# yitian97/SDformerFlow

Hardware: AMD Instinct MI355X
Metric: event-frames/sec fwd (1x10x2x288x384) (higher is better)
Workload: dtype f16x2

## Files before the change

include/sdformerflow_hip.h:

```cpp
#ifndef SDFORMERFLOW_HIP_H
#define SDFORMERFLOW_HIP_H

#include <stdint.h>

#ifdef __cplusplus
extern "C" {
#endif

#define SDF_VERSION 107

enum { SDF_F32 = 0, SDF_U8 = 1 };
enum { SDF_LIF = 0, SDF_PSN = 1, SDF_IF = 2 };
enum {
  SDF_E_NULL = -1,
  SDF_E_SHAPE = -2,
  SDF_E_DTYPE = -3,
  SDF_E_ALIGN = -4
};

int sdf_version(void);

void sdf_switches_reload(void);

typedef struct SdfLaunchRecord {
// ... 207 lines not shown

typedef struct SdfSpikeDeconvDesc {
  const uint8_t* spikes;
  const int8_t* digits; const float* cscale;
  const float* alpha; const float* beta;
  float* out;
  int32_t imgs, T, H, W, Cin, Cout;
} SdfSpikeDeconvDesc;

int sdf_spike_deconv3x3s2_fwd(const SdfSpikeDeconvDesc* d, void* stream);

typedef struct SdfSpikeConvDesc {
  SdfSpikeGemmDesc g;
  int32_t H, W, Cin, OH, OW;
  int32_t KH, KW, sy, sx;
  int32_t dy[3], dx[3];
} SdfSpikeConvDesc;

int sdf_spike_conv2d_fwd(const SdfSpikeConvDesc* c, void* stream);
int sdf_spike_conv2d_multi_fwd(const SdfSpikeConvDesc* cs, int n, void* stream);

int sdf_split_weight_bf16(const float* W, uint16_t* planes, int64_t n, int nsplit, void* stream);

int sdf_split_weight_f16x2(const float* W, uint16_t* planes, int64_t n, float scale, void* stream);

int sdf_qk_gate_fwd(const uint8_t* q, const uint8_t* k, uint8_t* e, int Tq, int64_t rows, int C,
                    int kind, float tau, float v_th, float v_reset, int soft_reset,
                    const float* psn_w, const float* psn_b, void* stream);
int sdf_qk_gate_strided_fwd(const uint8_t* q, const uint8_t* k, uint8_t* e, int Tq, int64_t rows, int C,
                            int64_t ldq, int64_t ldk, int kind, float tau, float v_th, float v_reset,
                            int soft_reset, const float* psn_w, const float* psn_b, void* stream);

typedef struct SdfHeadConvDesc {
  const float* x;
  const float* w;
  const float* alpha;
  const float* beta;
  uint8_t* out;
  int32_t B, T, H, W, Cin, Cout;
  int32_t sn_kind;
  float tau, v_th, v_reset;
  int32_t soft_reset;
  const float* psn_w;
  const float* psn_b;
  int64_t x_sb, x_st, x_sy, x_sx;
  int64_t x_sc[4];
} SdfHeadConvDesc;

int sdf_head_conv_sn_fwd(const SdfHeadConvDesc* d, void* stream);

typedef struct SdfPointwiseConvDesc {
  const float* x;
  const float* w;
  const float* bias;
  float* out;
  int32_t imgs, H, W, Cin, N, stride, OH, OW;
} SdfPointwiseConvDesc;

int sdf_pointwise_conv_f32_fwd(const SdfPointwiseConvDesc* d, void* stream);

int sdf_deconv_col2im_fwd(const float* Y, const float* alpha, const float* beta, float* out, int imgs, int H, int W,
                          int Cout, void* stream);

int sdf_flow_out_fwd(const float* pred, float* out, int B, int D, int h, int w, int64_t ldp, int C, int H, int W,
                     float scale_y, float scale_x, void* stream);

typedef struct SdfPredHeadDesc {
  const float* z;
  int32_t B, D, h, w, Cin;
  SdfNeuronCfg sn_pred;
  const float* wgt;
  const float* bias;
  float* pred;
  float* flow;
  int32_t H, W;
  uint8_t* next_spikes;
  int32_t next_ld, next_z_off, next_pred_off, next_zero_off, next_zero_len;
  SdfNeuronCfg sn_next;
  uint8_t* keep_spikes;
} SdfPredHeadDesc;

int sdf_pred_head_fwd(const SdfPredHeadDesc* d, void* stream);

int sdf_affine_resid_fwd(const float* x, const float* alpha, const float* beta, const float* resid, float* out,
                         int64_t n, int C, int64_t inner, void* stream);

enum { SDF_ATTN_ANN = 0, SDF_ATTN_SEW = 1 };
typedef struct SdfWinAttnDesc {
  int32_t mode;
  const void* q;
  const void* k;
  const void* v;
  float* out;
  int32_t B_, nW, nH, N, hd;
  int32_t Tq, N1;
  const float* scale;
  const float* bias;
  const float* mask;
  const int32_t* row_map;
  const float* pad_qkv;
} SdfWinAttnDesc;

int sdf_win_attn_fwd(const SdfWinAttnDesc* d, void* stream);

typedef struct SdfAnnAttnBlockDesc {
  const float* x;
  float* out;
  const int32_t* row_map;
  int32_t B_, nW, nH, N, C;
  int64_t rows;
  const float* ln_w;
  const float* ln_b;
  float ln_eps;
  const uint16_t* wqkv;
  const float* qkv_bias;
  const float* scale;
  const float* table;
  const uint16_t* wproj;
  const float* proj_bias;
} SdfAnnAttnBlockDesc;

int sdf_ann_attn_block_supported(int C, int nH, int N);
int sdf_ann_attn_block_fwd(const SdfAnnAttnBlockDesc* d, void* stream);

typedef struct SdfAnnMlpBlockDesc {
  const float* x;
  float* out;
  int64_t rows;
  int32_t C, Ch;
  const float* ln_w;
  const float* ln_b;
  float ln_eps;
  const uint16_t* w1;
  const float* b1;
  const uint16_t* w2;
  const float* b2;
} SdfAnnMlpBlockDesc;

int sdf_ann_mlp_block_supported(int C, int Ch);
int sdf_ann_mlp_block_fwd(const SdfAnnMlpBlockDesc* d, void* stream);

typedef struct SdfDenseConvDesc {
  const void* x;
  const uint16_t* w;
  const float* alpha;
  const float* beta;
  const void* resid;
  void* out;
  int32_t imgs, H, W, cin_records, N;
  int32_t relu;
  int32_t out_f32;
  int32_t x_records;
  float acc_scale;
} SdfDenseConvDesc;

int sdf_dense_conv3x3_fwd(const SdfDenseConvDesc* d, void* stream);
int sdf_pack_planes(const float* x, void* planes, int imgs, int C, int H, int W, void* stream);
int sdf_unpack_planes(const void* planes, float* x, int imgs, int C, int H, int W, void* stream);
int sdf_pack_planes_up2(const float* x, void* planes, int imgs, int C, int h, int w, int64_t sn, int64_t sc, int64_t sh, int64_t sw,
                        int rec0, int rec_total, void* stream);
int sdf_pack_planes_zero_up2(const float* x, void* planes, int imgs, int C, int h, int w, int64_t sn, int64_t sc, int64_t sh, int64_t sw,
                             int rec0, int rec_total, void* stream);

typedef struct SdfDenseLinearDesc {
  const float* a;
  const uint16_t* w;
// ... 45 lines not shown
```

sdformerflow_amd/csrc/pred_head.hip:

```cpp
#include "spike_mm.h"

namespace {
using sdfmm::neuron_T;

struct PredParams {
  SdfPredHeadDesc d;
  float inv_tau_p, inv_tau_n;
  int64_t P;
  int same_next;
};

template <int T, int LPP, int NK>
__global__ __launch_bounds__(256) void pred_head_kernel(PredParams P) {
  constexpr int Cin = 12 * LPP, PPW = 64 / LPP;
  const SdfPredHeadDesc& d = P.d;
  __shared__ __attribute__((aligned(16))) float psn_s[NK == 1 ? 2 * sdfmm::PSN_TABLE(T) : 4];
  if constexpr (NK == 1) {
    sdfmm::psn_stage<T>(psn_s, d.sn_pred, threadIdx.x, 256);
    if (d.next_spikes) sdfmm::psn_stage<T>(psn_s + sdfmm::PSN_TABLE(T), d.sn_next, threadIdx.x, 256);
    __syncthreads();
  }
  const int lane = threadIdx.x & 63, wave = threadIdx.x >> 6;
  const int g = lane % LPP, pw = lane / LPP;
  const int64_t pos = ((int64_t)blockIdx.x * 4 + wave) * PPW + pw;
  const bool ok = pos < P.P;
  const int64_t pc = ok ? pos : 0;
  const int64_t HW = (int64_t)d.h * d.w;
  const int64_t b = pc / HW, hw = pc - b * HW;
  const int64_t row0 = (b * T) * HW + hw;
  float acc[T][2];
#pragma unroll
  for (int t = 0; t < T; ++t) acc[t][0] = acc[t][1] = 0.f;
  const bool to_next = d.next_spikes != nullptr, keep = d.keep_spikes != nullptr;
  constexpr bool AHEAD = T <= 10;
  float4 vall[AHEAD ? 3 : 1][T];
  if (AHEAD) {
#pragma unroll
    for (int i = 0; i < 3; ++i)
#pragma unroll
      for (int t = 0; t < T; ++t) vall[AHEAD ? i : 0][t] = *reinterpret_cast<const float4*>(d.z + (row0 + t * HW) * Cin + 4 * (g + LPP * i));
  }
#pragma unroll
  for (int i = 0; i < 3; ++i) {
    const int c = 4 * (g + LPP * i);
    float4 v[T];
#pragma unroll
    for (int t = 0; t < T; ++t) v[t] = AHEAD ? vall[AHEAD ? i : 0][t] : *reinterpret_cast<const float4*>(d.z + (row0 + t * HW) * Cin + c);
    const float4 w0 = *reinterpret_cast<const float4*>(d.wgt + c), w1 = *reinterpret_cast<const float4*>(d.wgt + Cin + c);
    uint32_t pk[T], pk2[T];
#pragma unroll
    for (int t = 0; t < T; ++t) pk[t] = pk2[t] = 0;
#pragma unroll
    for (int e = 0; e < 4; ++e) {
      float xs[T], sp[T];
#pragma unroll
      for (int t = 0; t < T; ++t) xs[t] = e == 0 ? v[t].x : (e == 1 ? v[t].y : (e == 2 ? v[t].z : v[t].w));
      if constexpr (NK == 1) sdfmm::psn_T_lds<T>(xs, sp, psn_s); else neuron_T<NK, T>(xs, sp, d.sn_pred, P.inv_tau_p);
      const float we0 = e == 0 ? w0.x : (e == 1 ? w0.y : (e == 2 ? w0.z : w0.w));
      const float we1 = e == 0 ? w1.x : (e == 1 ? w1.y : (e == 2 ? w1.z : w1.w));
#pragma unroll
      for (int t = 0; t < T; ++t) {
        acc[t][0] = __builtin_fmaf(sp[t], we0, acc[t][0]);
        acc[t][1] = __builtin_fmaf(sp[t], we1, acc[t][1]);
        pk[t] |= ((__float_as_uint(sp[t]) >> 29) & 1u) << (8 * e);
      }
      if (to_next && !P.same_next) {
        if constexpr (NK == 1) sdfmm::psn_T_lds<T>(xs, sp, psn_s + sdfmm::PSN_TABLE(T)); else neuron_T<NK, T>(xs, sp, d.sn_next, P.inv_tau_n);
#pragma unroll
        for (int t = 0; t < T; ++t) pk2[t] |= ((__float_as_uint(sp[t]) >> 29) & 1u) << (8 * e);
      }
    }
    if (ok && keep) {
#pragma unroll
      for (int t = 0; t < T; ++t) *reinterpret_cast<uint32_t*>(d.keep_spikes + (row0 + t * HW) * Cin + c) = pk[t];
    }
    if (ok && to_next) {
#pragma unroll
      for (int t = 0; t < T; ++t)
        *reinterpret_cast<uint32_t*>(d.next_spikes + (row0 + t * HW) * d.next_ld + d.next_z_off + c) = P.same_next ? pk[t] : pk2[t];
    }
  }
#pragma unroll
  for (int m = 1; m < LPP; m <<= 1) {
#pragma unroll
    for (int t = 0; t < T; ++t) {
      acc[t][0] += __shfl_xor(acc[t][0], m, 64);
      acc[t][1] += __shfl_xor(acc[t][1], m, 64);
    }
  }
  const float b0 = d.bias ? d.bias[0] : 0.f, b1 = d.bias ? d.bias[1] : 0.f;
  float f0 = 0.f, f1 = 0.f;
#pragma unroll
  for (int t = 0; t < T; ++t) {
    acc[t][0] += b0; acc[t][1] += b1;
    f0 += acc[t][0]; f1 += acc[t][1];
  }
  if (!ok) return;
  if (g == 0) {
    if (d.pred) {
#pragma unroll
      for (int t = 0; t < T; ++t) *reinterpret_cast<float4*>(d.pred + (row0 + t * HW) * 4) = make_float4(acc[t][0], acc[t][1], 0.f, 0.f);
    }
    if (to_next) {
      float sp0[T], sp1[T], xs[T];
#pragma unroll
      for (int t = 0; t < T; ++t) xs[t] = acc[t][0];
      if constexpr (NK == 1) sdfmm::psn_T_lds<T>(xs, sp0, psn_s + sdfmm::PSN_TABLE(T)); else neuron_T<NK, T>(xs, sp0, d.sn_next, P.inv_tau_n);
#pragma unroll
      for (int t = 0; t < T; ++t) xs[t] = acc[t][1];
      if constexpr (NK == 1) sdfmm::psn_T_lds<T>(xs, sp1, psn_s + sdfmm::PSN_TABLE(T)); else neuron_T<NK, T>(xs, sp1, d.sn_next, P.inv_tau_n);
#pragma unroll
      for (int t = 0; t < T; ++t) {
        const uint32_t w = ((__float_as_uint(sp0[t]) >> 29) & 1u) | (((__float_as_uint(sp1[t]) >> 29) & 1u) << 8);
        uint8_t* dst = d.next_spikes + (row0 + t * HW) * d.next_ld;
        *reinterpret_cast<uint32_t*>(dst + d.next_pred_off) = w;
        for (int zo = 0; zo < d.next_zero_len; zo += 4) *reinterpret_cast<uint32_t*>(dst + d.next_zero_off + zo) = 0u;
      }
    }
  }
  if (d.flow) {
    const int sy = d.H / d.h, sx = d.W / d.w, blk = sy * sx;
    const int y = (int)(hw / d.w), x = (int)(hw - (int64_t)y * d.w);
    for (int i = g; i < 2 * blk; i += LPP) {
      const int o = i / blk, r = i - o * blk;
      const int dy = r / sx, dx = r - dy * sx;
      d.flow[((b * 2 + o) * d.H + (y * sy + dy)) * (int64_t)d.W + x * sx + dx] = o ? f1 : f0;
    }
  }
}

template <int T, int LPP>
int launch_nk(const PredParams& P, int nk, dim3 grid, hipStream_t s) {
  switch (nk) {
    case 0: SDF_LAUNCH((pred_head_kernel<T, LPP, 0>), grid, dim3(256), 0, s, P); return 0;
    case 1:
      if constexpr (T <= 10) { SDF_LAUNCH((pred_head_kernel<T, LPP, 1>), grid, dim3(256), 0, s, P); return 0; }
      return SDF_E_SHAPE;
    default: SDF_LAUNCH((pred_head_kernel<T, LPP, 2>), grid, dim3(256), 0, s, P); return 0;
  }
}

template <int T>
int launch_lpp(const PredParams& P, int nk, hipStream_t s) {
  const int lpp = P.d.Cin / 12;
  const int64_t per_wg = 4 * (64 / lpp), wgs = (P.P + per_wg - 1) / per_wg;
  if (wgs >= (1LL << 31)) return SDF_E_SHAPE;
  const dim3 grid((unsigned)wgs);
  switch (lpp) {
    case 8: return launch_nk<T, 8>(P, nk, grid, s);
    case 16: return launch_nk<T, 16>(P, nk, grid, s);
    case 32: return launch_nk<T, 32>(P, nk, grid, s);
    default: return SDF_E_SHAPE;
  }
}

bool same_neuron(const SdfNeuronCfg& a, const SdfNeuronCfg& b) {
  return a.kind == b.kind && a.tau == b.tau && a.v_th == b.v_th && a.v_reset == b.v_reset && a.soft_reset == b.soft_reset &&
         a.psn_w == b.psn_w && a.psn_b == b.psn_b;
}

int check_neuron(const SdfNeuronCfg& n) {
  if (n.kind != SDF_LIF && n.kind != SDF_PSN && n.kind != SDF_IF) return SDF_E_DTYPE;
  if (n.kind == SDF_PSN && (!n.psn_w || !n.psn_b)) return SDF_E_NULL;
  if (!sdf_tau_ok(n.kind, n.tau)) return SDF_E_SHAPE;
  return 0;
}
}

extern "C" int sdf_pred_head_fwd(const SdfPredHeadDesc* d, void* stream) {
  if (!d) return SDF_E_NULL;
  if (!d->z || !d->wgt) return SDF_E_NULL;
  if (!d->pred && !d->flow && !d->next_spikes) return SDF_E_NULL;
  if (d->B < 1 || d->h < 1 || d->w < 1) return SDF_E_SHAPE;
  if (d->Cin != 96 && d->Cin != 192 && d->Cin != 384) return SDF_E_SHAPE;
  if (d->D != 5 && d->D != 10 && d->D != 20) return SDF_E_SHAPE;
  int rc = check_neuron(d->sn_pred);
  if (rc) return rc;
  const int nk = sdfmm::neuron_class(d->sn_pred);
  if (nk == 1 && d->D > 10) return SDF_E_SHAPE;
  if (d->flow && (d->H < d->h || d->W < d->w || d->H % d->h || d->W % d->w)) return SDF_E_SHAPE;
  if (d->next_spikes) {
    rc = check_neuron(d->sn_next);
    if (rc) return rc;
    if (sdfmm::neuron_class(d->sn_next) != nk) return SDF_E_SHAPE;
    if (d->next_ld < 4 || d->next_ld % 4 || d->next_z_off % 4 || d->next_pred_off % 4 || d->next_zero_off % 4 || d->next_zero_len % 4 ||
        d->next_z_off < 0 || d->next_pred_off < 0 || d->next_zero_len < 0 || d->next_z_off + d->Cin > d->next_ld ||
        d->next_pred_off + 4 > d->next_ld || (d->next_zero_len > 0 && d->next_zero_off + d->next_zero_len > d->next_ld))
      return SDF_E_SHAPE;
    if (!sdf_aligned(d->next_spikes, 4)) return SDF_E_ALIGN;
  }
  if (!sdf_aligned(d->z, 16) || !sdf_aligned(d->wgt, 16) || (d->pred && !sdf_aligned(d->pred, 16)) ||
      (d->keep_spikes && !sdf_aligned(d->keep_spikes, 4)))
    return SDF_E_ALIGN;
  PredParams P;
  P.d = *d;
  P.inv_tau_p = sdfmm::inv_tau_of(d->sn_pred);
  P.inv_tau_n = d->next_spikes ? sdfmm::inv_tau_of(d->sn_next) : 0.f;
  P.P = (int64_t)d->B * d->h * d->w;
  P.same_next = d->next_spikes && same_neuron(d->sn_pred, d->sn_next);
  hipStream_t s = sdf_stream(stream);
  switch (d->D) {
    case 5: rc = launch_lpp<5>(P, nk, s); break;
    case 10: rc = launch_lpp<10>(P, nk, s); break;
    default: rc = launch_lpp<20>(P, nk, s); break;
  }
  if (rc) return rc;
  SDF_LAUNCH_CHECK();
  return 0;
}
```

sdformerflow_amd/csrc/switches.h:

```cpp
#pragma once
#define SDF_SWITCH_LIST(X)                                                                                                        \
  X(DENSE_TPW) X(DENSE_LINEAR_XCD) X(HEAD_MFMA) X(MLP_FUSED_ANY) X(MLP_FUSED) X(RES) X(RES_STRIP) X(RES_UPW) X(RES_RMUL)            \
  X(RES_MINC) X(RES_MAXC) X(SMALLM) X(SMALLM_CONV_ROWS) X(SMALLM_CB) X(SMALLM_FC2) X(WIDE) X(WIDE_CB) X(WIDE_PASSES)                \
  X(WIDE_MAXROWS) X(WIDE_CONV) X(QK_FRONT) X(QK_FRONT_ANY) X(CONV_WRES) X(CONV_WRES_RB) X(CONV_WRES_GROUPS) X(CONV_WRES_CB_INNER)   \
  X(CONV_WRES_NOSPK) X(CONV_MULTI) X(DECONV_WRES) X(DECONV_BALANCE) X(DECONV_EPI) X(GEMM_CFG) X(GEMM_WGS) X(PP_PAIR)     \
  X(ATTN_GENERIC) X(ATTN_F32) X(KSPLIT_MULT) X(GEMM_WS)
enum SdfSwitch {
#define X(n) SW_##n,
  SDF_SWITCH_LIST(X)
#undef X
      SW_COUNT
};
const char* sdf_sw(SdfSwitch s);
```

sdformerflow_amd/engine.py:

```python
from __future__ import annotations

import torch
import torch.nn.functional as F

from . import hip
from .STSwinNet_SNN.Spiking_swin_transformer3D import get_window_size, merge_row_map, window_slice_map

BN_EPS = 1e-5
_WIDE_MINC = 96


def bn_affine(bn, device):
    w, b = bn.weight.detach().float().cpu(), bn.bias.detach().float().cpu()
    m, v = bn.running_mean.detach().float().cpu(), bn.running_var.detach().float().cpu()
    alpha = w * torch.rsqrt(v + BN_EPS)
    beta = (b.double() - m.double() * alpha.double()).float()
    return alpha.contiguous().to(device), beta.contiguous().to(device)


class _Lin:

    def __init__(self, linear, bn, device, nsplit, digits=True):
        w = linear.weight.detach().float().to(device).contiguous()
        self.N, self.K = w.shape
# ... 556 lines not shown
            imgs.append(img)
            c1 = cout
        self._ready_has_y = len(calls) < 6
        if self._ready_has_y:
            cy, hw0, cp0 = y0.shape[-1], h0 * w0, imgs[0].shape[-1]
            calls.append((y0, imgs[0].view(-1), D, hw0, cy, cy, hw0 * cy, cp0, hw0 * cp0, self.decoders[0][2], None, 0, None, None, 0, 1, None, 0, 0,
                          None, (B, D * hw0 * cy, D * hw0 * cp0)))
        hip.neuron_multi_fwd(calls)
        return imgs

    def unet_tail(self, feats, out_size=None, s1=None):
        y = feats[-1]
        for i, rb in enumerate(self.unet_res):
            nxt = self.unet_res[i + 1].sn1 if i + 1 < len(self.unet_res) else None
            r = self._resblock(y, rb, s1=s1, next_sn=nxt)
            y, s1 = r if nxt is not None else (r, None)
        preds, E = [], len(feats)
        self._flows = [None] * E
        carried = None
        ready = self._prepare_decoder_images(feats, y, out_size) if self.tape is None else None
        for i in range(E):
            skip = feats[E - 1 - i]
            B, D, h, w, _ = skip.shape
            wdec, bn, sn = self.decoders[i]
            cout = wdec.shape[1]
            same = tuple(y.shape[2:4]) == (h, w)
            if same:
                C1, C2 = y.shape[-1], skip.shape[-1]
                cin = C1 + C2 + (4 if i > 0 else 0)
                as_gemm, cp = self._decoder_geometry(i, B, D, h, w, cin)
                if ready is not None:
                    s, c0 = ready[i], 0
                    srcs = [(y, C1, C1)] if i == 0 and not self._ready_has_y else []
                elif carried is not None:
                    s, srcs, c0 = carried, [(skip, C2, C2)], C1
                else:
                    s = (torch.zeros if cp != cin else torch.empty)((B, D, h, w, cp), dtype=torch.uint8, device=y.device)
                    srcs, c0 = [(y, C1, C1), (skip, C2, C2)] + ([(preds[-1], 4, preds[-1].shape[-1])] if i > 0 else []), 0
                hw = h * w
                for src, take, pitch in srcs:
                    for b in range(B):
                        hip.neuron_fwd(src[b], s[b].view(-1)[c0:], D, hw, take, pitch, hw * pitch, cp, hw * cp, sn)
                    c0 += take
                wkey = "perm"
                if self.tape is not None:
                    npred = self.preds[i - 1][3] if i > 0 else 0
                    self._rec(f"sttmultires_unet.decoders.{i}.sn.spiking_neuron.",
                              torch.cat([s[..., C1 + C2:C1 + C2 + npred], s[..., :C1 + C2]], -1), "BDHWC->TBCHW")
            else:
                parts = ([preds[-1][..., :self.preds[i - 1][3]]] if i > 0 else []) + [y, skip]
                parts = [F.pad(p, (0, 0, (w - p.shape[3]) // 2, w - p.shape[3] - (w - p.shape[3]) // 2,
                                   (h - p.shape[2]) // 2, h - p.shape[2] - (h - p.shape[2]) // 2)) for p in parts]
                cin = sum(p.shape[-1] for p in parts)
                as_gemm, cp = self._decoder_geometry(i, B, D, h, w, cin)
                cat = torch.zeros((B, D, h, w, cp), dtype=torch.float32, device=y.device) if cp != cin else None
                if cat is None:
                    cat = torch.cat(parts, dim=-1)
                else:
                    torch.cat(parts, dim=-1, out=cat[..., :cin])
                s = self._neuron_bd(cat, sn)
                wkey = "ref"
                self._rec(f"sttmultires_unet.decoders.{i}.sn.spiking_neuron.", s[..., :cin], "BDHWC->TBCHW")
            carried = None
            wuse = self._decoder_weight(i, wkey, y.shape[-1], skip.shape[-1])
            z = torch.empty((B, D, 2 * h, 2 * w, cout), dtype=torch.float32, device=y.device)
            if as_gemm:
                key = ("taps", i, cp, wkey)
                if key not in self._deconv:
                    self._deconv[key] = deconv_tap_weights(wuse, cp, self.nsplit)
                Y = torch.empty((B * D * h * w, 9 * cout), dtype=torch.float32, device=y.device)
                taps = self._deconv[key]
                M1, bc = self._rb(B) * D * h * w, B
                if getattr(taps, "digits", None) is not None and hip.smallm_gemm_applicable(M1, 9 * cout, cp):
                    taps = taps.digits
                    bc = max(n for n in range(1, B + 1) if B % n == 0 and hip.smallm_gemm_rows_ok(n * D * h * w))
                elif getattr(taps, "digits_rm", None) is not None and hip.res_gemm_applicable(M1, 9 * cout, cp):
                    taps = taps.digits_rm
                    bc = max(n for n in range(1, B + 1) if B % n == 0 and hip.res_gemm_applicable(n * D * h * w, 9 * cout, cp))
                if self.replicas and taps is self._deconv[key]:
                    bc = 1
                mc = bc * D * h * w
                for m0 in range(0, B * D * h * w, mc):
                    hip.spike_gemm(s.view(-1, cp)[m0:m0 + mc], taps, Y[m0:m0 + mc], mc, 9 * cout, cp)
                hip.deconv_col2im(Y, B * D, h, w, cout, alpha=bn[0], beta=bn[1], out=z)
            imgs = per = B * D
            fits = lambda n: n * 4 * h * w * cout * 4 < 1 << 31
            if not fits(per):
                whole = [n * D for n in range(B, 0, -1) if B % n == 0 and fits(n * D)]
                per = whole[0] if whole else per
            while not fits(per):
                per = (per + 1) // 2
            one_gemm = not as_gemm and self.nsplit == 2 and per % D == 0 and imgs % per == 0 and \
                hip.deconv2x2_applicable(per, D, h, w, cp, cout, fast_only=True)
            if one_gemm:
                key = ("d2x2", i, cp, wkey)
                if key not in self._deconv:
                    self._deconv[key] = (hip.pack_deconv2x2_weight(wuse, cp), bn[0].repeat(4).contiguous(), bn[1].repeat(4).contiguous())
                pl, a4, b4 = self._deconv[key]
                sv, zv = s.view(imgs, h, w, cp), z.view(imgs, 2 * h, 2 * w, cout)
                for i0 in range(0, imgs, per):
                    hip.spike_deconv3x3s2(sv[i0:i0 + per], pl, per, D, h, w, cp, cout, alpha=a4, beta=b4, out=zv[i0:i0 + per], tiled_bn=True)
            classes = [] if as_gemm or one_gemm else self._deconv_classes(i, B, D, h, w, cp, wkey, wuse)
            if classes and self.replicas and B > 1:
                c1 = self._deconv_classes(i, 1, D, h, w, cp, wkey, wuse)
                sv, zv = s.view(imgs, h, w, cp), z.view(imgs, 4 * h * w, cout)
                for b0 in range(0, imgs, D):
                    hip.spike_conv2d_multi(sv[b0:b0 + D], c1, D, h, w, cp, h, w, zv[b0:b0 + D], alpha=bn[0], beta=bn[1])
                classes = []
            if classes and per == imgs:
                hip.spike_conv2d_multi(s.view(imgs, h, w, cp), classes, imgs, h, w, cp, h, w, z.view(imgs, 4 * h * w, cout), alpha=bn[0], beta=bn[1])
                classes = []
            for cls in classes:
                for i0 in range(0, imgs, per):
                    n = min(per, imgs - i0)
                    hip.spike_conv2d(s.view(imgs, h, w, cp)[i0:i0 + n], cls["Wp"], n, h, w, cp, h, w, cls["KH"], cls["KW"], 1,
                                     cls["dy"], cls["dx"], out=z.view(imgs, 4 * h * w, cout)[i0:i0 + n], alpha=bn[0], beta=bn[1],
                                     out_rowmap=cls["rowmap"][:n * h * w])
            pw, pb, psn, nout, w2, b2 = self.preds[i]
            H2, W2 = 2 * h, 2 * w
            nxt_skip = feats[E - 2 - i] if i + 1 < E else None
            fs = out_size if out_size is not None and out_size[0] % H2 == 0 and out_size[1] % W2 == 0 else None
            if nout == 2 and hip.pred_head_supported(D, cout, fs[0] if fs else H2, fs[1] if fs else W2, H2, W2, psn,
                                                      self.decoders[i + 1][2] if nxt_skip is not None else None) \
                    and B * D * H2 * W2 * max(cout, 16) * 4 < 1 << 40:
                nxt = None
                if nxt_skip is not None and tuple(nxt_skip.shape[2:4]) == (H2, W2):
                    C1n, C2n = cout, nxt_skip.shape[-1]
                    cin_n = C1n + C2n + 4
                    _, cp_n = self._decoder_geometry(i + 1, B, D, H2, W2, cin_n)
                    carried = ready[i + 1] if ready is not None else torch.empty((B, D, H2, W2, cp_n), dtype=torch.uint8, device=y.device)
                    nxt = (carried, self.decoders[i + 1][2], 0, C1n + C2n, (cin_n, cp_n - cin_n))
                pred, flow, sp = hip.pred_head(z, w2, b2, psn, fs[0] if fs else None, fs[1] if fs else None,
                                               want_pred=self.tape is not None or fs is None or (i + 1 < E and nxt is None),
                                               nxt=nxt, keep=self.tape is not None)
                if sp is not None:
                    self._rec(f"sttmultires_unet.preds.{i}.sn.spiking_neuron.", sp, "BDHWC->TBCHW")
                self._flows[i] = flow
                preds.append(pred)
            else:
                sp = self._neuron_bd(z, psn)
                self._rec(f"sttmultires_unet.preds.{i}.sn.spiking_neuron.", sp, "BDHWC->TBCHW")
                po = torch.empty((B * D * 4 * h * w, 32), dtype=torch.float32, device=y.device)
                hip.spike_gemm(sp, pw, po, po.shape[0], 32, cout, bias=pb)
                preds.append(po.view(B, D, 2 * h, 2 * w, 32))
            y = z
        return [None if p is None else p[..., :self.preds[0][3]] for p in preds]

    def forward(self, x, scores=None, replicas=False):
        if not x.is_cuda:
            raise hip.SdfError("input must be a GPU tensor (no CPU fallback)")
        x = x.float().contiguous()
        H, W = x.shape[-2:]
        self.scores = scores
        if replicas and self.num_steps not in (10, 20):
            raise hip.ReplicaGeometryError(f"replicas are built for T = 10 / 20 (digit kernels throughout), not T = {self.num_steps}")
        self.replicas = bool(replicas)
        try:
            feats = self.encoder(x, **self._tail_kwargs())
            self.scores = None
            preds = self.unet_tail(feats, out_size=(H, W), **({"s1": self.tail_spikes} if getattr(self, "tail_spikes", None) is not None else {}))
        finally:
            self.scores = None
            self.replicas = False
        self.tail_spikes = None
        return [f if f is not None else hip.flow_out(p, H, W, H / p.shape[2], W / p.shape[3]) for p, f in zip(preds, self._flows)]
```

sdformerflow_amd/hip.py:

```python
from __future__ import annotations

import ctypes as C
import os

import torch

_HERE = os.path.dirname(os.path.abspath(__file__))
LIB_PATH = os.environ.get("SDF_HIP_LIB") or os.path.join(_HERE, "csrc", "libsdformerflow_hip.so")

SDF_F32, SDF_U8 = 0, 1
SDF_LIF, SDF_PSN, SDF_IF = 0, 1, 2
KIND = {"lif": SDF_LIF, "psn": SDF_PSN, "if": SDF_IF}

VOID_EXPORTS = ("sdf_switches_reload", "sdf_launch_log")
EXPORTS = ("sdf_version", "sdf_switches_reload", "sdf_launch_log", "sdf_launch_log_read", "sdf_lif_fwd", "sdf_psn_fwd", "sdf_neuron_fwd", "sdf_spike_gemm_fwd",
           "sdf_split_weight_bf16", "sdf_split_weight_f16x2", "sdf_qk_gate_fwd", "sdf_qk_gate_strided_fwd", "sdf_affine_resid_fwd", "sdf_win_attn_fwd", "sdf_ann_attn_block_fwd", "sdf_ann_attn_block_supported", "sdf_ann_mlp_block_fwd", "sdf_ann_mlp_block_supported", "sdf_spike_conv2d_fwd", "sdf_spike_deconv3x3s2_fwd", "sdf_head_conv_sn_fwd",
           "sdf_flow_out_fwd", "sdf_deconv_col2im_fwd", "sdf_lif_bwd", "sdf_psn_bwd", "sdf_psn_bwd_workspace_bytes",
           "sdf_window_slice_map", "sdf_window_zsrc_map", "sdf_qk_attn_fwd", "sdf_qk_attn_is_wide", "sdf_ms_mlp_is_wide", "sdf_ms_patch_merge_fwd", "sdf_tile_weight_i8x3", "sdf_spike_conv2d_multi_fwd", "sdf_qk_attn_workspace_bytes", "sdf_spike_gemm_bn_fwd",
           "sdf_ms_mlp_fwd", "sdf_ms_mlp_workspace_bytes", "sdf_pred_head_fwd", "sdf_pointwise_conv_f32_fwd", "sdf_neuron_multi_fwd", "sdf_qk_gate_f32_fwd", "sdf_qk_gate_bwd", "sdf_qk_gate_bwd_workspace_bytes",
           "sdf_rows_gather_fwd", "sdf_rows_scatter_fwd",
           "sdf_split_weight_i8x3", "sdf_bn_train_fwd", "sdf_bn_train_bwd", "sdf_bn_train_workspace_bytes", "sdf_bn_train_nchw_fwd", "sdf_bn_train_nchw_bwd",
           "sdf_dense_conv3x3_fwd", "sdf_pack_planes", "sdf_unpack_planes", "sdf_pack_planes_up2", "sdf_pack_planes_zero_up2", "sdf_dense_linear_fwd", "sdf_layer_norm_fwd",
           "sdf_linear_dw_fwd", "sdf_linear_dw_splits", "sdf_ringed_rows_fwd", "sdf_linear_train_fwd", "sdf_unring_rows_fwd")


class SdfError(RuntimeError):

    def __init__(self, msg, rc=None):
        super().__init__(msg)
        self.rc = rc


class ReplicaGeometryError(SdfError):
    """A replica launch sequence cannot serve this geometry (the window count per sample is not a multiple of the window depth at some
    stage): the caller runs the samples one by one - same results."""


_SW = {k: v for k, v in os.environ.items() if k.startswith("SDF_")}


def sw(name, default=None):
    return _SW.get(name, default)


def reload_switches():
    _SW.clear()
    _SW.update({k: v for k, v in os.environ.items() if k.startswith("SDF_")})
    if _lib is not None:
        _lib.sdf_switches_reload()


class scoped_switches:

    def __init__(self, **kw):
        self._kw = kw

    def __enter__(self):
        self._old = {k: os.environ.get(k) for k in self._kw}
        for k, v in self._kw.items():
            if v is None:
                os.environ.pop(k, None)
            else:
                os.environ[k] = str(v)
        reload_switches()
        return self

    def __exit__(self, *exc):
        for k, v in self._old.items():
            if v is None:
                os.environ.pop(k, None)
            else:
                os.environ[k] = v
        reload_switches()


class NeuronDesc(C.Structure):
    _fields_ = [("x", C.c_void_p), ("out", C.c_void_p), ("v_last", C.c_void_p),
                ("T", C.c_int32), ("out_dtype", C.c_int32),
                ("nb", C.c_int64), ("ni", C.c_int64),
                ("x_sb", C.c_int64), ("x_st", C.c_int64),
                ("o_sb", C.c_int64), ("o_st", C.c_int64),
                ("rowmap", C.c_void_p), ("rowlen", C.c_int32), ("kind", C.c_int32),
                ("alpha", C.c_void_p), ("beta", C.c_void_p), ("C", C.c_int32), ("inner", C.c_int32),
                ("add", C.c_void_p), ("add_st", C.c_int64), ("add_period", C.c_int64),
                ("tau", C.c_float), ("v_th", C.c_float), ("v_reset", C.c_float), ("soft_reset", C.c_int32),
                ("psn_w", C.c_void_p), ("psn_b", C.c_void_p),
                ("nrep", C.c_int64), ("x_srep", C.c_int64), ("o_srep", C.c_int64)]


class SpikeGemmDesc(C.Structure):
    _fields_ = [("A", C.c_void_p), ("Wp", C.c_void_p), ("out", C.c_void_p),
                ("M", C.c_int64), ("N", C.c_int32), ("K", C.c_int32),
                ("lda", C.c_int64), ("ldo", C.c_int64), ("nsplit", C.c_int32),
                ("bias", C.c_void_p), ("alpha", C.c_void_p), ("beta", C.c_void_p),
                ("resid", C.c_void_p), ("out_rowmap", C.c_void_p),
                ("zg_nH", C.c_int32), ("zg_T", C.c_int32), ("zg_B", C.c_int32), ("zg_N1", C.c_int32),
                ("sn_T", C.c_int32), ("sn_kind", C.c_int32),
                ("tau", C.c_float), ("v_th", C.c_float), ("v_reset", C.c_float), ("soft_reset", C.c_int32),
                ("psn_w", C.c_void_p), ("psn_b", C.c_void_p),
                ("pos_count", C.c_int64), ("pos_inner", C.c_int64), ("pos_ostride", C.c_int64), ("t_stride", C.c_int64),
                ("add", C.c_void_p), ("add_prows", C.c_int64), ("out_spike", C.c_void_p),
                ("workspace", C.c_void_p), ("workspace_bytes", C.c_int64), ("acc_scale", C.c_float), ("out_rows", C.c_int64),
# ... 1248 lines not shown
            d.x_sc[ci] = (ci // 2) * T * 2 * hw + (ci % 2) * hw
    d.x, d.w, d.out = _ptr(x, torch.float32), _ptr(w, torch.float32), _ptr(out, torch.uint8)
    d.alpha, d.beta = _ptr(alpha, torch.float32), _ptr(beta, torch.float32)
    d.B, d.T, d.H, d.W, d.Cin, d.Cout = B, T, H, W, Cin, Cout
    d.sn_kind, d.tau, d.v_th = KIND[p.kind], p.tau, p.v_th
    d.v_reset, d.soft_reset = (0.0 if p.v_reset is None else float(p.v_reset)), (1 if p.v_reset is None else 0)
    d.psn_w, d.psn_b = _ptr(p.psn_w, torch.float32), _ptr(p.psn_b, torch.float32)
    _check(lib().sdf_head_conv_sn_fwd(C.byref(d), _stream()), "sdf_head_conv_sn_fwd")
    return out


def flow_out(pred, H, W, scale_y, scale_x):
    B, D, h, w, Cc = pred.shape
    if pred.stride(4) != 1 or pred.stride(2) != w * pred.stride(3) or pred.stride(1) != h * pred.stride(2) or pred.stride(0) != D * pred.stride(1):
        raise SdfError("flow_out needs a (B,D,h,w,C) view of a dense (rows, ldp) buffer")
    out = torch.empty((B, Cc, H, W), dtype=torch.float32, device=pred.device)
    _check(lib().sdf_flow_out_fwd(C.c_void_p(_ptr(pred, torch.float32)), C.c_void_p(out.data_ptr()), C.c_int(B), C.c_int(D), C.c_int(h),
                                  C.c_int(w), C.c_int64(pred.stride(3)), C.c_int(Cc), C.c_int(H), C.c_int(W), C.c_float(scale_y),
                                  C.c_float(scale_x), _stream()), "sdf_flow_out_fwd")
    return out


class PointwiseConvDesc(C.Structure):
    _fields_ = [("x", C.c_void_p), ("w", C.c_void_p), ("bias", C.c_void_p), ("out", C.c_void_p), ("imgs", C.c_int32), ("H", C.c_int32),
                ("W", C.c_int32), ("Cin", C.c_int32), ("N", C.c_int32), ("stride", C.c_int32), ("OH", C.c_int32), ("OW", C.c_int32)]


def pointwise_conv_supported(Cin, N):
    return Cin == 96 and N in (96, 192)


def pointwise_conv_f32(x, w, stride, bias=None):
    imgs, H, W, Cin = x.shape
    N = w.shape[0]
    if not x.is_contiguous() or not w.is_contiguous() or tuple(w.shape) != (N, Cin):
        raise SdfError("pointwise_conv_f32 needs a contiguous NHWC image and an (N, Cin) weight")
    OH, OW = (H - 1) // stride + 1, (W - 1) // stride + 1
    out = torch.empty((imgs, OH, OW, N), dtype=torch.float32, device=x.device)
    d = PointwiseConvDesc()
    d.x, d.w, d.bias, d.out = _ptr(x, torch.float32), _ptr(w, torch.float32), _ptr(bias, torch.float32), out.data_ptr()
    d.imgs, d.H, d.W, d.Cin, d.N, d.stride, d.OH, d.OW = imgs, H, W, Cin, N, stride, OH, OW
    _check(lib().sdf_pointwise_conv_f32_fwd(C.byref(d), _stream()), "sdf_pointwise_conv_f32_fwd")
    return out


class PredHeadDesc(C.Structure):
    _fields_ = [("z", C.c_void_p), ("B", C.c_int32), ("D", C.c_int32), ("h", C.c_int32), ("w", C.c_int32), ("Cin", C.c_int32),
                ("sn_pred", NeuronCfg), ("wgt", C.c_void_p), ("bias", C.c_void_p), ("pred", C.c_void_p), ("flow", C.c_void_p),
                ("H", C.c_int32), ("W", C.c_int32), ("next_spikes", C.c_void_p), ("next_ld", C.c_int32), ("next_z_off", C.c_int32),
                ("next_pred_off", C.c_int32), ("next_zero_off", C.c_int32), ("next_zero_len", C.c_int32), ("sn_next", NeuronCfg),
                ("keep_spikes", C.c_void_p)]


def pred_head_supported(D, Cin, H, W, h, w, sn, sn_next=None):
    if Cin not in (96, 192, 384) or D not in (5, 10, 20) or H % h or W % w:
        return False
    if sn.kind == "psn" and D > 10:
        return False
    return sn_next is None or sn_next.kind == sn.kind or {sn.kind, sn_next.kind} <= {"lif", "if"}


def pred_head(z, wgt, bias, sn, H, W, want_pred=True, nxt=None, keep=False):
    B, D, h, w, Cin = z.shape
    d = PredHeadDesc()
    d.z, d.B, d.D, d.h, d.w, d.Cin = _ptr(z, torch.float32), B, D, h, w, Cin
    _ncfg(d.sn_pred, sn)
    d.wgt, d.bias = _ptr(wgt, torch.float32), _ptr(bias, torch.float32)
    pred = torch.empty((B, D, h, w, 4), dtype=torch.float32, device=z.device) if want_pred else None
    flow = torch.empty((B, 2, H, W), dtype=torch.float32, device=z.device) if H is not None else None
    d.pred, d.flow, d.H, d.W = _ptr(pred), _ptr(flow), H or 0, W or 0
    if nxt is not None:
        img, sn_next, z_off, p_off, (zero_off, zero_len) = nxt
        if img.dtype != torch.uint8 or not img.is_contiguous() or tuple(img.shape[:4]) != (B, D, h, w):
            raise SdfError("the next level's spike image must be a contiguous (B,D,h,w,ld) u8 tensor")
        d.next_spikes, d.next_ld, d.next_z_off, d.next_pred_off = img.data_ptr(), img.shape[4], z_off, p_off
        d.next_zero_off, d.next_zero_len = zero_off, zero_len
        _ncfg(d.sn_next, sn_next)
    sp = torch.empty((B, D, h, w, Cin), dtype=torch.uint8, device=z.device) if keep else None
    d.keep_spikes = _ptr(sp)
    _check(lib().sdf_pred_head_fwd(C.byref(d), _stream()), "sdf_pred_head_fwd")
    return pred, flow, sp


def deconv2x2_applicable(imgs, T, H, W, Cin, Cout, fast_only=False):
    if sw("SDF_DECONV_GEMM", "1") == "0" or sw("SDF_RES", "1") == "0":
        return False
    rows = imgs * H * W
    ok = T in (10, 20) and imgs % T == 0 and Cin % 16 == 0 and 16 <= Cin <= 256 and Cout % 8 == 0 and Cout >= 8 and \
        rows * Cin < 1 << 31 and rows * 16 * Cout < 1 << 31
    if fast_only:
        ok = ok and Cin == 208 and rows >= 4096 and sw("SDF_DECONV_WRES", "1") != "0"
    return ok


def pack_deconv2x2_weight(w, cin_pad):
    Cin, Cout = w.shape[:2]
    w = w.detach().float()
    M = torch.zeros((4 * Cout, 4 * cin_pad), dtype=torch.float32, device=w.device)
    tap = {(0, 0): 1, (1, 0): 2, (1, 1): 0}
    for py in range(2):
        for px in range(2):
            for dh in range(2):
                for dw in range(2):
                    if (py, dh) in tap and (px, dw) in tap:
                        q, cls = dh + 2 * dw, 2 * py + px
                        M[cls * Cout:(cls + 1) * Cout, q * cin_pad:q * cin_pad + Cin] = w[:, :, tap[(py, dh)], tap[(px, dw)]].t()
    return split_weight_i8x3(M)


def spike_deconv3x3s2(s, planes, imgs, T, H, W, Cin, Cout, alpha=None, beta=None, out=None, tiled_bn=False):
    if out is None:
        out = torch.empty((imgs, 2 * H, 2 * W, Cout), dtype=torch.float32, device=s.device)
    d = SpikeDeconvDesc()
    d.spikes, d.digits, d.cscale = _ptr(s, torch.uint8), _ptr(planes, torch.int8), _ptr(planes.sdf_col_scale, torch.float32)
    if alpha is not None and not tiled_bn:
        alpha, beta = alpha.repeat(4).contiguous(), beta.repeat(4).contiguous()
    d.alpha, d.beta = _ptr(alpha, torch.float32), _ptr(beta, torch.float32)
    d.out, d.imgs, d.T, d.H, d.W, d.Cin, d.Cout = _ptr(out, torch.float32), imgs, T, H, W, Cin, Cout
    _check(lib().sdf_spike_deconv3x3s2_fwd(C.byref(d), _stream()), "sdf_spike_deconv3x3s2_fwd")
    return out


def deconv_col2im(Y, imgs, H, W, Cout, alpha=None, beta=None, out=None):
    if out is None:
        out = torch.empty((imgs, 2 * H, 2 * W, Cout), dtype=torch.float32, device=Y.device)
    _check(lib().sdf_deconv_col2im_fwd(C.c_void_p(_ptr(Y, torch.float32)), C.c_void_p(_ptr(alpha, torch.float32)),
                                       C.c_void_p(_ptr(beta, torch.float32)), C.c_void_p(_ptr(out, torch.float32)), C.c_int(imgs),
                                       C.c_int(H), C.c_int(W), C.c_int(Cout), _stream()), "sdf_deconv_col2im_fwd")
    return out
```

Measured before the change: 844.3.

## Fuse deconv col2im gather and BN affine into the prediction head kernel

```diff
diff --git a/include/sdformerflow_hip.h b/include/sdformerflow_hip.h
--- a/include/sdformerflow_hip.h
+++ b/include/sdformerflow_hip.h
@@ -313,6 +313,15 @@
 
 int sdf_pred_head_fwd(const SdfPredHeadDesc* d, void* stream);
 
+typedef struct SdfDeconvPredHeadDesc {
+  const float* Y;
+  const float* alpha;
+  const float* beta;
+  SdfPredHeadDesc head;
+} SdfDeconvPredHeadDesc;
+
+int sdf_deconv_pred_head_fwd(const SdfDeconvPredHeadDesc* d, void* stream);
+
 int sdf_affine_resid_fwd(const float* x, const float* alpha, const float* beta, const float* resid, float* out,
                          int64_t n, int C, int64_t inner, void* stream);
 
diff --git a/sdformerflow_amd/csrc/pred_head.hip b/sdformerflow_amd/csrc/pred_head.hip
--- a/sdformerflow_amd/csrc/pred_head.hip
+++ b/sdformerflow_amd/csrc/pred_head.hip
@@ -1,4 +1,5 @@
 #include "spike_mm.h"
+#include "switches.h"
 
 namespace {
 using sdfmm::neuron_T;
@@ -8,9 +9,57 @@
   float inv_tau_p, inv_tau_n;
   int64_t P;
   int same_next;
+  const float* Y;
+  const float* alpha;
+  const float* beta;
 };
 
-template <int T, int LPP, int NK>
+template <int T>
+__device__ __forceinline__ void col2im_z(const PredParams& P, int64_t b, int oy, int ox, int c, float4 (&z)[T]) {
+  const int Hi = P.d.h >> 1, Wi = P.d.w >> 1, Cout = P.d.Cin;
+  const int y0 = oy >> 1, x0 = ox >> 1;
+  const int ny = (oy & 1) ? ((y0 + 1 < Hi) ? 2 : 1) : 1, nx = (ox & 1) ? ((x0 + 1 < Wi) ? 2 : 1) : 1;
+  const int64_t ldy = 9 * (int64_t)Cout, img_st = (int64_t)Hi * Wi * ldy;
+#pragma unroll
+  for (int t = 0; t < T; ++t) z[t] = make_float4(0.f, 0.f, 0.f, 0.f);
+#pragma unroll
+  for (int a = 0; a < 2; ++a) {
+    if (a < ny) {
+      const int iy = y0 + a, ky = (oy & 1) ? (a == 0 ? 2 : 0) : 1, kx0 = (ox & 1) ? 2 : 1;
+      const float* p0 = P.Y + ((b * T * Hi + iy) * Wi + x0) * ldy + (ky * 3 + kx0) * Cout + c;
+      constexpr bool BOTH = T <= 10;
+      float4 v0[T], v1[T];
+#pragma unroll
+      for (int t = 0; t < T; ++t) v0[t] = *reinterpret_cast<const float4*>(p0 + t * img_st);
+      if (BOTH && nx == 2) {
+        const float* p1 = p0 + ldy + (0 - kx0) * Cout;
+#pragma unroll
+        for (int t = 0; t < T; ++t) v1[t] = *reinterpret_cast<const float4*>(p1 + t * img_st);
+      }
+#pragma unroll
+      for (int t = 0; t < T; ++t) { z[t].x += v0[t].x; z[t].y += v0[t].y; z[t].z += v0[t].z; z[t].w += v0[t].w; }
+      if (nx == 2) {
+        if (!BOTH) {
+          const float* p1 = p0 + ldy + (0 - kx0) * Cout;
+#pragma unroll
+          for (int t = 0; t < T; ++t) v1[t] = *reinterpret_cast<const float4*>(p1 + t * img_st);
+        }
+#pragma unroll
+        for (int t = 0; t < T; ++t) { z[t].x += v1[t].x; z[t].y += v1[t].y; z[t].z += v1[t].z; z[t].w += v1[t].w; }
+      }
+    }
+  }
+  if (P.alpha) {
+    const float4 al = *reinterpret_cast<const float4*>(P.alpha + c), be = *reinterpret_cast<const float4*>(P.beta + c);
+#pragma unroll
+    for (int t = 0; t < T; ++t) {
+      z[t].x = __builtin_fmaf(z[t].x, al.x, be.x); z[t].y = __builtin_fmaf(z[t].y, al.y, be.y);
+      z[t].z = __builtin_fmaf(z[t].z, al.z, be.z); z[t].w = __builtin_fmaf(z[t].w, al.w, be.w);
+    }
+  }
+}
+
+template <int T, int LPP, int NK, bool FY>
 __global__ __launch_bounds__(256) void pred_head_kernel(PredParams P) {
   constexpr int Cin = 12 * LPP, PPW = 64 / LPP;
   const SdfPredHeadDesc& d = P.d;
@@ -26,13 +75,21 @@
   const bool ok = pos < P.P;
   const int64_t pc = ok ? pos : 0;
   const int64_t HW = (int64_t)d.h * d.w;
-  const int64_t b = pc / HW, hw = pc - b * HW;
+  const int64_t b = pc / HW;
+  int64_t hw = pc - b * HW;
+  int oy = 0, ox = 0;
+  if constexpr (FY) {
+    oy = (int)(hw / d.w);
+    const int r = (int)(hw - (int64_t)oy * d.w), half = d.w >> 1;
+    ox = r < half ? 2 * r : 2 * (r - half) + 1;
+    hw = (int64_t)oy * d.w + ox;
+  }
   const int64_t row0 = (b * T) * HW + hw;
   float acc[T][2];
 #pragma unroll
   for (int t = 0; t < T; ++t) acc[t][0] = acc[t][1] = 0.f;
   const bool to_next = d.next_spikes != nullptr, keep = d.keep_spikes != nullptr;
-  constexpr bool AHEAD = T <= 10;
+  constexpr bool AHEAD = T <= 10 && !FY;
   float4 vall[AHEAD ? 3 : 1][T];
   if (AHEAD) {
 #pragma unroll
@@ -44,8 +101,12 @@
   for (int i = 0; i < 3; ++i) {
     const int c = 4 * (g + LPP * i);
     float4 v[T];
-#pragma unroll
-    for (int t = 0; t < T; ++t) v[t] = AHEAD ? vall[AHEAD ? i : 0][t] : *reinterpret_cast<const float4*>(d.z + (row0 + t * HW) * Cin + c);
+    if constexpr (FY) {
+      col2im_z<T>(P, b, oy, ox, c, v);
+    } else {
+#pragma unroll
+      for (int t = 0; t < T; ++t) v[t] = AHEAD ? vall[AHEAD ? i : 0][t] : *reinterpret_cast<const float4*>(d.z + (row0 + t * HW) * Cin + c);
+    }
     const float4 w0 = *reinterpret_cast<const float4*>(d.wgt + c), w1 = *reinterpret_cast<const float4*>(d.wgt + Cin + c);
     uint32_t pk[T], pk2[T];
 #pragma unroll
@@ -129,27 +190,27 @@
   }
 }
 
-template <int T, int LPP>
+template <int T, int LPP, bool FY>
 int launch_nk(const PredParams& P, int nk, dim3 grid, hipStream_t s) {
   switch (nk) {
-    case 0: SDF_LAUNCH((pred_head_kernel<T, LPP, 0>), grid, dim3(256), 0, s, P); return 0;
+    case 0: SDF_LAUNCH((pred_head_kernel<T, LPP, 0, FY>), grid, dim3(256), 0, s, P); return 0;
     case 1:
-      if constexpr (T <= 10) { SDF_LAUNCH((pred_head_kernel<T, LPP, 1>), grid, dim3(256), 0, s, P); return 0; }
+      if constexpr (T <= 10) { SDF_LAUNCH((pred_head_kernel<T, LPP, 1, FY>), grid, dim3(256), 0, s, P); return 0; }
       return SDF_E_SHAPE;
-    default: SDF_LAUNCH((pred_head_kernel<T, LPP, 2>), grid, dim3(256), 0, s, P); return 0;
-  }
-}
-
-template <int T>
+    default: SDF_LAUNCH((pred_head_kernel<T, LPP, 2, FY>), grid, dim3(256), 0, s, P); return 0;
+  }
+}
+
+template <int T, bool FY>
 int launch_lpp(const PredParams& P, int nk, hipStream_t s) {
   const int lpp = P.d.Cin / 12;
   const int64_t per_wg = 4 * (64 / lpp), wgs = (P.P + per_wg - 1) / per_wg;
   if (wgs >= (1LL << 31)) return SDF_E_SHAPE;
   const dim3 grid((unsigned)wgs);
   switch (lpp) {
-    case 8: return launch_nk<T, 8>(P, nk, grid, s);
-    case 16: return launch_nk<T, 16>(P, nk, grid, s);
-    case 32: return launch_nk<T, 32>(P, nk, grid, s);
+    case 8: return launch_nk<T, 8, FY>(P, nk, grid, s);
+    case 16: return launch_nk<T, 16, FY>(P, nk, grid, s);
+    case 32: return launch_nk<T, 32, FY>(P, nk, grid, s);
     default: return SDF_E_SHAPE;
   }
 }
@@ -165,11 +226,8 @@
   if (!sdf_tau_ok(n.kind, n.tau)) return SDF_E_SHAPE;
   return 0;
 }
-}
-
-extern "C" int sdf_pred_head_fwd(const SdfPredHeadDesc* d, void* stream) {
-  if (!d) return SDF_E_NULL;
-  if (!d->z || !d->wgt) return SDF_E_NULL;
+int check_head(const SdfPredHeadDesc* d) {
+  if (!d->wgt) return SDF_E_NULL;
   if (!d->pred && !d->flow && !d->next_spikes) return SDF_E_NULL;
   if (d->B < 1 || d->h < 1 || d->w < 1) return SDF_E_SHAPE;
   if (d->Cin != 96 && d->Cin != 192 && d->Cin != 384) return SDF_E_SHAPE;
@@ -189,22 +247,55 @@
       return SDF_E_SHAPE;
     if (!sdf_aligned(d->next_spikes, 4)) return SDF_E_ALIGN;
   }
-  if (!sdf_aligned(d->z, 16) || !sdf_aligned(d->wgt, 16) || (d->pred && !sdf_aligned(d->pred, 16)) ||
-      (d->keep_spikes && !sdf_aligned(d->keep_spikes, 4)))
+  if (!sdf_aligned(d->wgt, 16) || (d->pred && !sdf_aligned(d->pred, 16)) || (d->keep_spikes && !sdf_aligned(d->keep_spikes, 4)))
     return SDF_E_ALIGN;
-  PredParams P;
-  P.d = *d;
+  return 0;
+}
+
+template <bool FY>
+int launch_head(PredParams& P, hipStream_t s) {
+  const SdfPredHeadDesc* d = &P.d;
+  const int nk = sdfmm::neuron_class(d->sn_pred);
   P.inv_tau_p = sdfmm::inv_tau_of(d->sn_pred);
   P.inv_tau_n = d->next_spikes ? sdfmm::inv_tau_of(d->sn_next) : 0.f;
   P.P = (int64_t)d->B * d->h * d->w;
   P.same_next = d->next_spikes && same_neuron(d->sn_pred, d->sn_next);
-  hipStream_t s = sdf_stream(stream);
+  int rc;
   switch (d->D) {
-    case 5: rc = launch_lpp<5>(P, nk, s); break;
-    case 10: rc = launch_lpp<10>(P, nk, s); break;
-    default: rc = launch_lpp<20>(P, nk, s); break;
+    case 5: rc = launch_lpp<5, FY>(P, nk, s); break;
+    case 10: rc = launch_lpp<10, FY>(P, nk, s); break;
+    default: rc = launch_lpp<20, FY>(P, nk, s); break;
   }
   if (rc) return rc;
   SDF_LAUNCH_CHECK();
   return 0;
 }
+}
+
+extern "C" int sdf_pred_head_fwd(const SdfPredHeadDesc* d, void* stream) {
+  if (!d) return SDF_E_NULL;
+  if (!d->z) return SDF_E_NULL;
+  int rc = check_head(d);
+  if (rc) return rc;
+  if (!sdf_aligned(d->z, 16)) return SDF_E_ALIGN;
+  PredParams P;
+  P.d = *d;
+  P.Y = P.alpha = P.beta = nullptr;
+  return launch_head<false>(P, sdf_stream(stream));
+}
+
+extern "C" int sdf_deconv_pred_head_fwd(const SdfDeconvPredHeadDesc* d, void* stream) {
+  if (!d) return SDF_E_NULL;
+  if (!d->Y) return SDF_E_NULL;
+  if (d->alpha && !d->beta) return SDF_E_NULL;
+  if (const char* e = sdf_sw(SW_DECONV_HEAD)) if (e[0] == '0') return SDF_E_SHAPE;
+  int rc = check_head(&d->head);
+  if (rc) return rc;
+  if (d->head.h % 2 || d->head.w % 2) return SDF_E_SHAPE;
+  if (!sdf_aligned(d->Y, 16) || (d->alpha && (!sdf_aligned(d->alpha, 16) || !sdf_aligned(d->beta, 16)))) return SDF_E_ALIGN;
+  PredParams P;
+  P.d = d->head;
+  P.d.z = nullptr;
+  P.Y = d->Y; P.alpha = d->alpha; P.beta = d->beta;
+  return launch_head<true>(P, sdf_stream(stream));
+}
diff --git a/sdformerflow_amd/csrc/switches.h b/sdformerflow_amd/csrc/switches.h
--- a/sdformerflow_amd/csrc/switches.h
+++ b/sdformerflow_amd/csrc/switches.h
@@ -3,7 +3,7 @@
   X(DENSE_TPW) X(DENSE_LINEAR_XCD) X(HEAD_MFMA) X(MLP_FUSED_ANY) X(MLP_FUSED) X(RES) X(RES_STRIP) X(RES_UPW) X(RES_RMUL)            \
   X(RES_MINC) X(RES_MAXC) X(SMALLM) X(SMALLM_CONV_ROWS) X(SMALLM_CB) X(SMALLM_FC2) X(WIDE) X(WIDE_CB) X(WIDE_PASSES)                \
   X(WIDE_MAXROWS) X(WIDE_CONV) X(QK_FRONT) X(QK_FRONT_ANY) X(CONV_WRES) X(CONV_WRES_RB) X(CONV_WRES_GROUPS) X(CONV_WRES_CB_INNER)   \
-  X(CONV_WRES_NOSPK) X(CONV_MULTI) X(DECONV_WRES) X(DECONV_BALANCE) X(DECONV_EPI) X(GEMM_CFG) X(GEMM_WGS) X(PP_PAIR)     \
+  X(CONV_WRES_NOSPK) X(CONV_MULTI) X(DECONV_WRES) X(DECONV_BALANCE) X(DECONV_EPI) X(DECONV_HEAD) X(GEMM_CFG) X(GEMM_WGS) X(PP_PAIR)     \
   X(ATTN_GENERIC) X(ATTN_F32) X(KSPLIT_MULT) X(GEMM_WS)
 enum SdfSwitch {
 #define X(n) SW_##n,
diff --git a/sdformerflow_amd/engine.py b/sdformerflow_amd/engine.py
--- a/sdformerflow_amd/engine.py
+++ b/sdformerflow_amd/engine.py
@@ -662,7 +662,8 @@
                 mc = bc * D * h * w
                 for m0 in range(0, B * D * h * w, mc):
                     hip.spike_gemm(s.view(-1, cp)[m0:m0 + mc], taps, Y[m0:m0 + mc], mc, 9 * cout, cp)
-                hip.deconv_col2im(Y, B * D, h, w, cout, alpha=bn[0], beta=bn[1], out=z)
+            else:
+                Y = None
             imgs = per = B * D
             fits = lambda n: n * 4 * h * w * cout * 4 < 1 << 31
             if not fits(per):
@@ -710,14 +711,26 @@
                     _, cp_n = self._decoder_geometry(i + 1, B, D, H2, W2, cin_n)
                     carried = ready[i + 1] if ready is not None else torch.empty((B, D, H2, W2, cp_n), dtype=torch.uint8, device=y.device)
                     nxt = (carried, self.decoders[i + 1][2], 0, C1n + C2n, (cin_n, cp_n - cin_n))
-                pred, flow, sp = hip.pred_head(z, w2, b2, psn, fs[0] if fs else None, fs[1] if fs else None,
-                                               want_pred=self.tape is not None or fs is None or (i + 1 < E and nxt is None),
-                                               nxt=nxt, keep=self.tape is not None)
+                want_pred = self.tape is not None or fs is None or (i + 1 < E and nxt is None)
+                if Y is not None and (nxt is not None or i + 1 == E) and self.tape is None and \
+                        hip.deconv_pred_head_applicable(D, cout, fs[0] if fs else H2, fs[1] if fs else W2, H2, W2, psn,
+                                                        nxt[1] if nxt else None):
+                    pred, flow = hip.deconv_pred_head(Y, bn[0], bn[1], B, D, h, w, cout, w2, b2, psn, fs[0] if fs else None,
+                                                      fs[1] if fs else None, want_pred=want_pred, nxt=nxt)
+                    sp = Y = None
+                else:
+                    if Y is not None:
+                        hip.deconv_col2im(Y, B * D, h, w, cout, alpha=bn[0], beta=bn[1], out=z)
+                        Y = None
+                    pred, flow, sp = hip.pred_head(z, w2, b2, psn, fs[0] if fs else None, fs[1] if fs else None,
+                                                   want_pred=want_pred, nxt=nxt, keep=self.tape is not None)
                 if sp is not None:
                     self._rec(f"sttmultires_unet.preds.{i}.sn.spiking_neuron.", sp, "BDHWC->TBCHW")
                 self._flows[i] = flow
                 preds.append(pred)
             else:
+                if Y is not None:
+                    hip.deconv_col2im(Y, B * D, h, w, cout, alpha=bn[0], beta=bn[1], out=z)
                 sp = self._neuron_bd(z, psn)
                 self._rec(f"sttmultires_unet.preds.{i}.sn.spiking_neuron.", sp, "BDHWC->TBCHW")
                 po = torch.empty((B * D * 4 * h * w, 32), dtype=torch.float32, device=y.device)
diff --git a/sdformerflow_amd/hip.py b/sdformerflow_amd/hip.py
--- a/sdformerflow_amd/hip.py
+++ b/sdformerflow_amd/hip.py
@@ -17,7 +17,7 @@
            "sdf_split_weight_bf16", "sdf_split_weight_f16x2", "sdf_qk_gate_fwd", "sdf_qk_gate_strided_fwd", "sdf_affine_resid_fwd", "sdf_win_attn_fwd", "sdf_ann_attn_block_fwd", "sdf_ann_attn_block_supported", "sdf_ann_mlp_block_fwd", "sdf_ann_mlp_block_supported", "sdf_spike_conv2d_fwd", "sdf_spike_deconv3x3s2_fwd", "sdf_head_conv_sn_fwd",
            "sdf_flow_out_fwd", "sdf_deconv_col2im_fwd", "sdf_lif_bwd", "sdf_psn_bwd", "sdf_psn_bwd_workspace_bytes",
            "sdf_window_slice_map", "sdf_window_zsrc_map", "sdf_qk_attn_fwd", "sdf_qk_attn_is_wide", "sdf_ms_mlp_is_wide", "sdf_ms_patch_merge_fwd", "sdf_tile_weight_i8x3", "sdf_spike_conv2d_multi_fwd", "sdf_qk_attn_workspace_bytes", "sdf_spike_gemm_bn_fwd",
-           "sdf_ms_mlp_fwd", "sdf_ms_mlp_workspace_bytes", "sdf_pred_head_fwd", "sdf_pointwise_conv_f32_fwd", "sdf_neuron_multi_fwd", "sdf_qk_gate_f32_fwd", "sdf_qk_gate_bwd", "sdf_qk_gate_bwd_workspace_bytes",
+           "sdf_ms_mlp_fwd", "sdf_ms_mlp_workspace_bytes", "sdf_pred_head_fwd", "sdf_deconv_pred_head_fwd", "sdf_pointwise_conv_f32_fwd", "sdf_neuron_multi_fwd", "sdf_qk_gate_f32_fwd", "sdf_qk_gate_bwd", "sdf_qk_gate_bwd_workspace_bytes",
            "sdf_rows_gather_fwd", "sdf_rows_scatter_fwd",
            "sdf_split_weight_i8x3", "sdf_bn_train_fwd", "sdf_bn_train_bwd", "sdf_bn_train_workspace_bytes", "sdf_bn_train_nchw_fwd", "sdf_bn_train_nchw_bwd",
            "sdf_dense_conv3x3_fwd", "sdf_pack_planes", "sdf_unpack_planes", "sdf_pack_planes_up2", "sdf_pack_planes_zero_up2", "sdf_dense_linear_fwd", "sdf_layer_norm_fwd",
@@ -1432,6 +1432,37 @@
     return pred, flow, sp
 
 
+class DeconvPredHeadDesc(C.Structure):
+    _fields_ = [("Y", C.c_void_p), ("alpha", C.c_void_p), ("beta", C.c_void_p), ("head", PredHeadDesc)]
+
+
+def deconv_pred_head_applicable(D, Cout, H, W, h, w, sn, sn_next=None):
+    return sw("SDF_DECONV_HEAD", "1") != "0" and h % 2 == 0 and w % 2 == 0 and pred_head_supported(D, Cout, H, W, h, w, sn, sn_next)
+
+
+def deconv_pred_head(Y, alpha, beta, B, D, h, w, Cout, wgt, bias, sn, H, W, want_pred=True, nxt=None):
+    d = DeconvPredHeadDesc()
+    d.Y, d.alpha, d.beta = _ptr(Y, torch.float32), _ptr(alpha, torch.float32), _ptr(beta, torch.float32)
+    hd, h2, w2 = d.head, 2 * h, 2 * w
+    hd.z, hd.B, hd.D, hd.h, hd.w, hd.Cin = None, B, D, h2, w2, Cout
+    _ncfg(hd.sn_pred, sn)
+    hd.wgt, hd.bias = _ptr(wgt, torch.float32), _ptr(bias, torch.float32)
+    pred = torch.empty((B, D, h2, w2, 4), dtype=torch.float32, device=Y.device) if want_pred else None
+    flow = torch.empty((B, 2, H, W), dtype=torch.float32, device=Y.device) if H is not None else None
+    hd.pred, hd.flow, hd.H, hd.W = _ptr(pred), _ptr(flow), H or 0, W or 0
+    if nxt is not None:
+        img, sn_next, z_off, p_off, (zero_off, zero_len) = nxt
+        if img.dtype != torch.uint8 or not img.is_contiguous() or tuple(img.shape[:4]) != (B, D, h2, w2):
+            raise SdfError("the next level's spike image must be a contiguous (B,D,h,w,ld) u8 tensor")
+        hd.next_spikes, hd.next_ld, hd.next_z_off, hd.next_pred_off = img.data_ptr(), img.shape[4], z_off, p_off
+        hd.next_zero_off, hd.next_zero_len = zero_off, zero_len
+        _ncfg(hd.sn_next, sn_next)
+    if tuple(Y.shape) != (B * D * h * w, 9 * Cout) or not Y.is_contiguous():
+        raise SdfError("Y must be a contiguous (B*D*h*w, 9*Cout) fp32 tensor")
+    _check(lib().sdf_deconv_pred_head_fwd(C.byref(d), _stream()), "sdf_deconv_pred_head_fwd")
+    return pred, flow
+
+
 def deconv2x2_applicable(imgs, T, H, W, Cin, Cout, fast_only=False):
     if sw("SDF_DECONV_GEMM", "1") == "0" or sw("SDF_RES", "1") == "0":
         return False
```

After: 858.1 (median of 6 runs). +1.6%, better.
